# UltimateSoftware/surge

Measured on NVIDIA H100. Metric: events/sec replayed (segmented per-aggregate event fold), higher is better.
Workload: dtype i32

## Files before the change

### include/sgr.h

```cpp
#ifndef SGR_H
#define SGR_H

#include <stddef.h>
#include <stdint.h>

#ifdef __cplusplus
extern "C" {
#endif

#define SGR_ABI_VERSION 1

#define SGR_OK                 0
#define SGR_ERR_INVALID       -1
#define SGR_ERR_NO_DEVICE     -2
#define SGR_ERR_CUDA          -3
#define SGR_ERR_NO_PROGRAM    -4
#define SGR_ERR_NOT_LOADED    -5
#define SGR_ERR_UNSUPPORTED   -6
#define SGR_ERR_OOM           -7
#define SGR_ERR_STATE         -8
#define SGR_ERR_DIST          -9
#define SGR_ERR_CAPACITY     -10
#define SGR_ERR_AGAIN        -11

// ... 46 lines not shown

typedef struct sgr_engine sgr_engine;

typedef struct sgr_config {
  int32_t  device;
  uint32_t flags;
  uint64_t reserved[6];
} sgr_config;

typedef struct sgr_stats {
  uint64_t n_aggregates;
  uint64_t n_events;
  uint64_t event_bytes;
  uint64_t algorithmic_bytes;
  uint64_t n_errors;
  uint64_t n_long_segments;
  float    ms_h2d;
  float    ms_group;
  float    ms_fold;
  float    ms_d2h;
  uint32_t fold_launches;
  uint32_t head_plane;
  uint32_t plane_bytes;
  uint32_t reserved[5];
} sgr_stats;

int32_t sgr_abi_version(void);

int32_t sgr_create(const sgr_config* cfg, sgr_engine** out);
int32_t sgr_destroy(sgr_engine* e);
const char* sgr_last_error(const sgr_engine* e);

int32_t sgr_register_program(sgr_engine* e, const sgr_fold_program* prog);

int32_t sgr_load_events(sgr_engine* e, const void* events, uint64_t nbytes,
                        const uint64_t* seg_offsets, uint64_t n_agg);
int32_t sgr_load_events_device(sgr_engine* e, const void* d_events, uint64_t nbytes,
                               const uint64_t* d_seg_offsets, uint64_t n_agg);

int32_t sgr_load_events_indexed(sgr_engine* e, const void* events, uint64_t nbytes, const uint64_t* seg_offsets, uint64_t n_agg,
                                const uint64_t* rec_offsets, uint64_t n_records);
int32_t sgr_load_events_indexed_device(sgr_engine* e, const void* d_events, uint64_t nbytes, const uint64_t* d_seg_offsets,
                                       uint64_t n_agg, const uint64_t* d_rec_offsets, uint64_t n_records);

int32_t sgr_load_unsorted(sgr_engine* e, const void* records, uint64_t n_records, uint64_t n_agg);
int32_t sgr_load_unsorted_device(sgr_engine* e, const void* d_records, uint64_t n_records, uint64_t n_agg);

// ... 180 lines not shown
```

### surge_b200/csrc/engine.cu

```cuda
#include <cuda_runtime.h>
#include <stdarg.h>
#include <stdio.h>
#include <string.h>

#include <atomic>
#include <memory>
#include <mutex>
#include <string>
#include <vector>

#include "../../include/sgr.h"
#include "bulk_fold.cuh"
#include "changes.cuh"
#include "devbuf.h"
#include "dist.cuh"
#include "engine_internal.h"
#include "fold_kernels.cuh"
#include "fold_rows.cuh"
#include "group_kernels.cuh"
#include "id_index.cuh"
#include "id_order.cuh"
#include "incremental.cuh"
#include "keytable.h"
#include "put_batch.cuh"
// ... 16 lines not shown
constexpr size_t kCtlDup = 0, kCtlNoSlot = 1, kCtlGatherBad = 2, kCtlCut = 4, kCtlRange = 8, kPayloadOff = 96;

struct FlaggedRows {
  enum Kind { kWholeTable, kNothing, kHostList, kDeviceList };
  Kind kind = kWholeTable;
  uint64_t n = 0;
  uint32_t upper = 0;
  int next = 0;
  void forget() { kind = kWholeTable; }
  void nothing() { kind = kNothing; }
  void host_list(uint64_t count) { kind = kHostList; n = count; }
  void device_list(uint32_t bound) { kind = kDeviceList; upper = bound; next ^= 1; }
};

struct PendingFold {
  enum Kernel { kSequential, kRows, kRuns, kVarRuns };
  Kernel kernel = kSequential;
  bool stamped = false;
  bool prior = false;
  uint64_t n_seg = 0, event_bytes = 0;
  const uint8_t* events = nullptr; const uint64_t* offsets = nullptr; const uint32_t* ids = nullptr;
  const void* counters = nullptr;
  uint32_t plane = 0;
};
}

struct sgr_engine {
  int device = 0;
  int num_sms = 0;
  Stream stream;
  Event ev0, ev1;

  bool has_program = false;
  sgr_fold_program program{};
  DevProgram dprog{};

  DevBuf own_events, own_offsets, own_rec_offsets;
  const uint64_t* d_rec_offsets = nullptr;
  uint64_t n_rec = 0;
  const uint8_t* d_events = nullptr;
  const uint64_t* d_offsets = nullptr;
  uint64_t event_bytes = 0;
  uint64_t n_agg = 0;
  bool loaded = false;
  uint32_t max_record_bytes = 64;

  DevBuf states;
  bool states_valid = false;
  uint64_t states_n = 0;
  DevBuf counters;
  GroupScratch group;
  DevBuf inc_records, inc_offsets, inc_ids, inc_prev_ids;
  DevBuf inc_scratch, inc_touched[2], inc_err_ids, inc_counters;
  uint64_t inc_scratch_slots = 0;
  FlaggedRows flagged;

  bool row_ok = false;
  RowProgram row_prog{};
  int row_max_grid = 0;
  int run_max_grid = 0, run_max_grid_variant = -2, run_max_grid_plane = -2;
  int64_t opt_run_variant = -1;
  DevBuf part_flags, part_data, redo_ids;
  DevBuf run_counters;
  int run_counter_idx = 0;
  int64_t opt_run_chunk_bytes = 131072;
  uint32_t epoch = 0;
  size_t part_flags_cap_seen = 0;
  bool offsets_aligned64 = false;
  uint64_t log_begin = 0, log_end = 0, max_seg_bytes = 0;
  DevBuf head_plane;
  enum PlaneState { kPlaneNone, kPlaneValid, kPlaneNoMemory } plane_state = kPlaneNone;
  uint32_t plane_bytes = 0;
  int64_t opt_head_plane = 1;
  int64_t opt_head_variant = -1;
  int64_t opt_proj_variant = 0;
  Stream side_stream;
  Event ev_copied, ev_split;
  bool fold_pending = false;
  PendingFold pending;
  Event ev2, ev3;

  int64_t opt_kernel = 0;
  int64_t opt_variant = -1;
  int64_t opt_var_stages = 1;
  int64_t opt_var_stage_bytes = 12288;
  int64_t opt_replay_budget = 1ll << 24;
  int64_t opt_force_route = 0;
  int64_t opt_incremental = 0;
  int64_t opt_max_record_bytes = 528;

  bool bulk_ok = false;
  BulkLayout bulk_lay{};
  DevBuf bulk_scratch, bulk_err_ids, bulk_counters, hash_out;
  uint64_t bulk_scratch_slots = 0;
  int64_t opt_bulk = 1;
  int64_t opt_push_ordered = 0;
  int64_t opt_push_chunks = 16;

// ... 113 lines not shown
  return SGR_OK;
}

int32_t refresh_snapshot(sgr_engine* e, std::shared_ptr<Snapshot>* out) {
  std::lock_guard<std::recursive_mutex> g(e->op_mu);
  if (!e->snapshot_dirty.load(std::memory_order_acquire) && e->snapshot) { *out = e->snapshot; return SGR_OK; }
  const uint64_t gen = e->generation.load(std::memory_order_acquire);
  if (!e->states_valid) return fail(e, SGR_ERR_STATE, "state store is not readable: no fold has completed");
  int32_t rc = use_device(e); if (rc) return rc;
  rc = finish_fold(e); if (rc) return rc;
  auto s = std::make_shared<Snapshot>();
  s->n_agg = e->states_n; s->state_bytes = e->program.state_bytes;
  s->states.resize((size_t)s->n_agg * s->state_bytes);
  CUDA_TRY(e, cudaMemcpyAsync(s->states.data(), e->states.p, s->states.size(), cudaMemcpyDeviceToHost, e->stream));
  CUDA_TRY(e, cudaStreamSynchronize(e->stream));
  std::atomic_store(&e->snapshot, s);
  if (e->generation.load(std::memory_order_acquire) == gen) e->snapshot_dirty.store(false, std::memory_order_release);
  *out = s;
  return SGR_OK;
}

constexpr uint64_t kRedoCap = 1u << 20;

int32_t begin_lookback(sgr_engine* e, uint64_t n_warps_max, uint64_t words) {
  CUDA_TRY(e, e->part_flags.reserve(n_warps_max * 4 + 256));
  CUDA_TRY(e, e->part_data.reserve(n_warps_max * words * 4 + 256));
  CUDA_TRY(e, e->redo_ids.reserve(kRedoCap * 4));
  if (e->epoch == 0 || e->part_flags_cap_seen != e->part_flags.cap) {
    CUDA_TRY(e, cudaMemsetAsync(e->part_flags.p, 0, e->part_flags.cap, e->stream));
    e->part_flags_cap_seen = e->part_flags.cap;
  }
  ++e->epoch;
  if (e->epoch == 0) { CUDA_TRY(e, cudaMemsetAsync(e->part_flags.p, 0, e->part_flags.cap, e->stream)); e->epoch = 1; }
  return SGR_OK;
}

int32_t launch_replay(sgr_engine* e, const uint8_t* d_events, const uint64_t* d_offsets, const uint32_t* d_ids, const uint8_t* states_in,
                      unsigned long long* counters) {
  FoldArgs a{};
  a.events = d_events; a.seg_offsets = d_offsets; a.seg_ids = d_ids; a.n_seg = kRedoCap; a.seg_list = (const uint32_t*)e->redo_ids.p;
  a.n_seg_dev = counters + 3; a.states_in = states_in; a.states_out = (uint8_t*)e->states.p; a.counters = counters;
  FoldLaunchInfo info{};
  cudaError_t le = launch_fold_stream(a, e->dprog, -1, 8, e->max_record_bytes, e->stream, &info);
  if (le != cudaSuccess) return fail(e, SGR_ERR_CUDA, "replay launch: %s", cudaGetErrorString(le));
  return SGR_OK;
}

bool plane_wanted(const sgr_engine* e) {
  return e->row_ok && e->row_prog.head_only && e->opt_head_plane && e->opt_kernel == 0 && e->opt_run_variant < 0 &&
         e->program.record_kind == SGR_REC_FIXED64 && e->offsets_aligned64 && e->log_end > e->log_begin;
}

uint32_t plane_record_bytes(const sgr_engine* e) { return slot_plane_fits(e->row_prog) && e->opt_head_variant < 0 ? 16u : 32u; }

cudaError_t build_plane(sgr_engine* e, const uint8_t* log, uint32_t rec, uint64_t r0, uint64_t r1, cudaStream_t st) {
  uint8_t* p = (uint8_t*)e->head_plane.p;
  return rec == 16 ? launch_build_slots(log, p, r0, r1, e->row_prog, e->num_sms, st) : launch_build_heads(log, p, r0, r1, e->num_sms, st);
}

int32_t ensure_plane(sgr_engine* e, uint32_t* plane, bool* built) {
  const uint32_t rec = plane_record_bytes(e);
  *plane = 0; *built = false;
  if (e->plane_bytes != rec) e->plane_state = sgr_engine::kPlaneNone;
  if (e->plane_state == sgr_engine::kPlaneValid) *plane = rec;
  if (e->plane_state != sgr_engine::kPlaneNone) return SGR_OK;
  e->plane_bytes = rec;
  const uint64_t n_rec = (e->log_end - e->log_begin) / 64;
  if (e->fold_pending && e->head_plane.cap < n_rec * rec) CUDA_TRY(e, cudaStreamSynchronize(e->stream));
  if (e->head_plane.reserve(n_rec * rec) != cudaSuccess) {
    (void)cudaGetLastError();
    e->plane_state = sgr_engine::kPlaneNoMemory;
    return SGR_OK;
  }
  cudaError_t le = build_plane(e, e->d_events + e->log_begin, rec, 0, n_rec, e->stream);
  if (le != cudaSuccess) return fail(e, SGR_ERR_CUDA, "plane build: %s", cudaGetErrorString(le));
  e->plane_state = sgr_engine::kPlaneValid;
  *plane = rec; *built = true;
  return SGR_OK;
}

int32_t enqueue_fold(sgr_engine* e, const uint8_t* d_events, const uint64_t* d_offsets, const uint32_t* d_ids,
                     uint64_t n_seg, bool use_prior, uint64_t event_bytes, bool aligned64, uint64_t log_begin, uint64_t log_end) {
  const uint8_t* states_in = use_prior ? (const uint8_t*)e->states.p : nullptr;
  const bool wide_balanced = e->row_prog.user_words == 14 && e->opt_kernel == 0 && d_offsets == e->d_offsets && e->max_seg_bytes <= (256u << 10);
  bool use_rows = e->row_ok && !wide_balanced && e->program.record_kind == SGR_REC_FIXED64 && aligned64 && e->opt_kernel != 1 && n_seg < (1ull << 32) && n_seg > 0;
  if ((e->opt_kernel == 2 || e->opt_kernel == 3) && !use_rows && n_seg > 0)
    return fail(e, SGR_ERR_UNSUPPORTED, "record-parallel kernel cannot take this program/log");
  if (use_rows && e->opt_kernel == 3 && (e->row_prog.user_words != 2 || e->row_prog.cls != 0 || e->row_prog.n_slots > 6 || e->row_prog.f64_mask))
    return fail(e, SGR_ERR_UNSUPPORTED, "the record-per-lane kernel takes 16-byte class-0 programs only");
  const bool runs = use_rows && e->opt_kernel != 3;
  uint32_t plane = 0;
  bool plane_built = false;
  if (runs && plane_wanted(e) && d_events == e->d_events && d_offsets == e->d_offsets && !d_ids) {
    int32_t rc = ensure_plane(e, &plane, &plane_built); if (rc) return rc;
  }
  unsigned long long* counters = (unsigned long long*)e->counters.p;
  if (runs) {
    if (!e->run_counters.p) {
      CUDA_TRY(e, e->run_counters.reserve(256));
      CUDA_TRY(e, cudaMemsetAsync(e->run_counters.p, 0, 256, e->stream));
    }
    counters = (unsigned long long*)e->run_counters.p + 16 * e->run_counter_idx;
  } else {
    CUDA_TRY(e, cudaMemsetAsync(e->counters.p, 0, 64, e->stream));
  }
  const bool overlap = runs && !plane_built && e->fold_pending && e->pending.kernel == PendingFold::kRuns && e->pending.events == d_events &&
                       e->pending.offsets == d_offsets && e->pending.ids == d_ids && e->pending.plane == plane;
  if (!overlap) CUDA_TRY(e, cudaEventRecord(e->ev0, e->stream));
  uint32_t launches = 0;
  PendingFold::Kernel kernel = PendingFold::kSequential;
  const bool use_var = e->row_ok && e->row_prog.user_words == 2 && e->row_prog.cls == 0 && e->program.record_kind == SGR_REC_VAR16 && e->d_rec_offsets && d_offsets == e->d_offsets && !use_prior &&
                       !d_ids && e->opt_kernel != 1 && n_seg > 0 && n_seg < (1ull << 32) && e->n_rec > 0;
  if (use_var) {
    int threads = 0; size_t smem = 0; uint32_t stage = 0;
    const int max_grid = vruns_config(e->num_sms, e->max_record_bytes, (uint32_t)e->opt_var_stage_bytes, (int)e->opt_var_stages, &threads, &smem, &stage);
    if (max_grid > 0) {
      int32_t rc = begin_lookback(e, (uint64_t)max_grid * (threads / 32), 8); if (rc) return rc;
      CUDA_TRY(e, cudaMemsetAsync(e->states.p, 0, (size_t)n_seg * e->program.state_bytes, e->stream));
      VarArgs v{};
      v.events = d_events; v.rec_offsets = e->d_rec_offsets; v.n_rec = e->n_rec; v.seg_offsets = d_offsets; v.n_seg = n_seg;
      v.states_out = (uint8_t*)e->states.p; v.counters = counters; v.redo_ids = (uint32_t*)e->redo_ids.p; v.redo_cap = kRedoCap;
      v.part_flags = (uint32_t*)e->part_flags.p; v.part_data = (uint32_t*)e->part_data.p; v.epoch = e->epoch; v.stage_bytes = stage;
      v.max_record_bytes = e->max_record_bytes;
      const uint64_t steps = (e->n_rec + 31) / 32;
      uint64_t want = (steps + (threads / 32) - 1) / (threads / 32);
      const int grid = (int)(want < (uint64_t)max_grid ? want : (uint64_t)max_grid);
      cudaError_t le = launch_fold_vruns(v, e->row_prog, (int)e->opt_var_stages, grid, threads, smem, e->stream);
      if (le != cudaSuccess) return fail(e, SGR_ERR_CUDA, "fold_vruns launch: %s", cudaGetErrorString(le));
      rc = launch_replay(e, d_events, d_offsets, d_ids, states_in, counters); if (rc) return rc;
      launches = 2;
      kernel = PendingFold::kVarRuns;
    }
  }
  if (n_seg && kernel != PendingFold::kVarRuns) {
    if (use_rows) {
      const bool v1 = e->opt_kernel == 3;
      const int rv = plane == 16 ? (int)e->opt_proj_variant : plane == 32 ? (e->opt_head_variant < 0 ? 0 : (int)e->opt_head_variant)
                                                                          : (int)e->opt_run_variant;
      const int pl = (int)plane;
      if (v1 && !e->row_max_grid) e->row_max_grid = row_kernel_max_grid(e->num_sms, e->row_prog);
      if (!v1 && (e->run_max_grid_variant != rv || e->run_max_grid_plane != pl)) {
        e->run_max_grid = run_kernel_max_grid(e->num_sms, rv, pl, e->row_prog); e->run_max_grid_variant = rv; e->run_max_grid_plane = pl;
      }
      const int max_grid = v1 ? e->row_max_grid : e->run_max_grid;
      const int wpc = v1 ? kRowThreads / 32 : run_warps_per_cta();
      const uint64_t step_bytes = v1 ? 2048 : (uint64_t)run_variant_step_bytes(rv, pl, e->row_prog);
      const uint64_t steps = (log_end - log_begin + step_bytes - 1) / step_bytes;
      const uint64_t chunk_steps = v1 ? 1 : run_variant_chunk_steps(rv, pl, e->row_prog, (uint64_t)e->opt_run_chunk_bytes, steps, (uint64_t)max_grid * wpc);
      const uint64_t n_chunks = (steps + chunk_steps - 1) / chunk_steps;
      const uint64_t n_parts = v1 ? (uint64_t)max_grid * wpc : n_chunks;
      int32_t rc = begin_lookback(e, n_parts, e->row_prog.user_words + 2); if (rc) return rc;
      RowArgs r{};
      r.events = d_events; r.heads = plane ? (const uint8_t*)e->head_plane.p : nullptr; r.seg_offsets = d_offsets; r.seg_ids = d_ids; r.n_seg = n_seg;
      r.log_begin = log_begin; r.log_end = log_end;
      r.states_in = states_in; r.states_out = (uint8_t*)e->states.p;
      r.counters = counters;
      r.counters_next = runs ? (unsigned long long*)e->run_counters.p + 16 * (e->run_counter_idx ^ 1) : nullptr;
      r.redo_ids = (uint32_t*)e->redo_ids.p; r.redo_cap = kRedoCap;
      r.part_flags = (uint32_t*)e->part_flags.p; r.part_data = (uint32_t*)e->part_data.p; r.epoch = e->epoch;
      r.chunk_steps = chunk_steps;
      uint64_t want = (n_chunks + wpc - 1) / wpc;
      if (want == 0) want = 1;
      const int grid = (int)(want < (uint64_t)max_grid ? want : (uint64_t)max_grid);
      cudaError_t le = v1 ? launch_fold_rows(r, e->row_prog, grid, e->stream) : launch_fold_runs(r, e->row_prog, rv, pl, grid, overlap, e->stream);
      if (le != cudaSuccess) return fail(e, SGR_ERR_CUDA, "fold launch: %s", cudaGetErrorString(le));
      if (runs) {
        e->run_counter_idx ^= 1;
        launches = 1;
      } else {
        rc = launch_replay(e, d_events, d_offsets, d_ids, states_in, counters); if (rc) return rc;
        launches = 2;
      }
      kernel = runs ? PendingFold::kRuns : PendingFold::kRows;
    } else {
      FoldArgs a{};
      a.events = d_events; a.seg_offsets = d_offsets; a.seg_ids = d_ids; a.n_seg = n_seg;
      a.states_in = states_in; a.states_out = (uint8_t*)e->states.p;
      a.counters = counters;
      FoldLaunchInfo info{};
      cudaError_t le = launch_fold_stream(a, e->dprog, (int)e->opt_variant, e->num_sms, e->max_record_bytes, e->stream, &info);
      if (le == cudaErrorNotSupported || le == cudaErrorInvalidConfiguration)
        return fail(e, SGR_ERR_UNSUPPORTED, "fold_variant %lld cannot take this program at max_record_bytes %u (%s)",
                    (long long)e->opt_variant, e->max_record_bytes, cudaGetErrorString(le));
      if (le != cudaSuccess) return fail(e, SGR_ERR_CUDA, "fold launch: %s", cudaGetErrorString(le));
      launches = 1;
    }
  }
  if (!overlap) CUDA_TRY(e, cudaEventRecord(e->ev1, e->stream));
  e->fold_pending = true;
  e->pending = PendingFold{kernel, overlap, use_prior, n_seg, event_bytes, d_events, d_offsets, d_ids, counters, plane};
  e->stats.fold_launches = launches;
  e->stats.head_plane = plane ? 1u : 0u;
  e->stats.plane_bytes = plane;
  return SGR_OK;
}

int32_t finish_fold(sgr_engine* e) {
  if (!e->fold_pending) return SGR_OK;
  e->fold_pending = false;
  PendingFold& p = e->pending;
  unsigned long long h[16] = {};
  CUDA_TRY(e, cudaMemcpyAsync(h, p.counters, p.kernel == PendingFold::kRuns ? 128 : 64, cudaMemcpyDeviceToHost, e->stream));
  CUDA_TRY(e, cudaStreamSynchronize(e->stream));
  if (p.stamped) e->stats.ms_fold = (h[8] && h[9] > ~h[8]) ? (float)((double)(h[9] - ~h[8]) * 1e-6) : 0.f;
  else CUDA_TRY(e, cudaEventElapsedTime(&e->stats.ms_fold, e->ev0, e->ev1));
  if ((p.kernel == PendingFold::kVarRuns && h[7]) || (p.kernel != PendingFold::kSequential && h[3] > kRedoCap)) {
    if (p.prior) {
      e->states_valid = false; mark_dirty(e);
      return fail(e, SGR_ERR_UNSUPPORTED, "replay list overflow on an in-place incremental fold: state table invalidated, rebuild it");
    }
    FoldArgs a{};
    a.events = p.events; a.seg_offsets = p.offsets; a.seg_ids = p.ids; a.n_seg = p.n_seg;
    a.states_out = (uint8_t*)e->states.p; a.counters = (unsigned long long*)e->counters.p;
    CUDA_TRY(e, cudaMemsetAsync(e->counters.p, 0, 64, e->stream));
    CUDA_TRY(e, cudaEventRecord(e->ev2, e->stream));
    FoldLaunchInfo info{};
// ... 59 lines not shown
  *out = e.release();
  return SGR_OK;
}

int32_t sgr_destroy(sgr_engine* e) {
  if (!e) return SGR_OK;
  cudaSetDevice(e->device);
  cudaStreamSynchronize(e->stream);
  delete e;
  return SGR_OK;
}

int32_t sgr_register_program(sgr_engine* e, const sgr_fold_program* prog) {
  OpLock op_lock(e);
  if (!e || !prog) return fail(e, SGR_ERR_INVALID, "null argument");
  DevProgram d;
  int32_t rc = compile_program(e, prog, &d);
  if (rc) return rc;
  e->program = *prog; e->dprog = d; e->has_program = true;
  e->row_ok = build_row_program(d, &e->row_prog);
  e->bulk_ok = e->row_ok && prog->record_kind == SGR_REC_FIXED64 && bulk_layout_for(e->row_prog, &e->bulk_lay);
  e->bulk_scratch_slots = 0;
  e->row_max_grid = 0; e->run_max_grid_variant = -2;
  e->plane_state = sgr_engine::kPlaneNone;
  e->states_valid = false; e->states_n = 0;
  e->writer.n = 0;
  e->writer_framing = SGR_VALUE_JSON;
  mark_dirty(e);
  return SGR_OK;
}

static int32_t before_load(sgr_engine* e) {
  int32_t rc = use_device(e); if (rc) return rc;
  return finish_fold(e);
}

struct Upload { void* dst; const void* src; size_t bytes; };

static int32_t upload_timed(sgr_engine* e, cudaEvent_t t0, cudaEvent_t t1, std::initializer_list<Upload> uploads) {
  CUDA_TRY(e, cudaEventRecord(t0, e->stream));
  for (const Upload& u : uploads) CUDA_TRY(e, cudaMemcpyAsync(u.dst, u.src, u.bytes, cudaMemcpyHostToDevice, e->stream));
  CUDA_TRY(e, cudaEventRecord(t1, e->stream));
  CUDA_TRY(e, cudaStreamSynchronize(e->stream));
  CUDA_TRY(e, cudaEventElapsedTime(&e->stats.ms_h2d, t0, t1));
  return SGR_OK;
}

static int32_t after_load(sgr_engine* e, const uint8_t* d_events, const uint64_t* d_offsets, uint64_t nbytes, uint64_t n_agg) {
  e->d_events = d_events; e->d_offsets = d_offsets; e->event_bytes = nbytes; e->n_agg = n_agg; e->loaded = true;
  e->d_rec_offsets = nullptr; e->n_rec = 0;
  e->max_record_bytes = e->program.record_kind == SGR_REC_VAR16 ? (uint32_t)e->opt_max_record_bytes : 64u;
  e->offsets_aligned64 = false; e->log_begin = 0; e->log_end = nbytes;
  e->plane_state = sgr_engine::kPlaneNone;
  if (e->program.record_kind == SGR_REC_FIXED64) {
    cudaError_t ce = inspect_offsets(d_offsets, n_agg, (unsigned long long*)e->counters.p, e->stream, &e->offsets_aligned64,
                                     &e->log_begin, &e->log_end, &e->max_seg_bytes);
    if (ce != cudaSuccess) return fail(e, SGR_ERR_CUDA, "offset inspection: %s", cudaGetErrorString(ce));
  }
  return SGR_OK;
}

int32_t sgr_load_events(sgr_engine* e, const void* events, uint64_t nbytes, const uint64_t* seg_offsets, uint64_t n_agg) {
  OpLock op_lock(e);
  if (!e || (!events && nbytes) || !seg_offsets) return fail(e, SGR_ERR_INVALID, "null argument");
  if (!e->has_program) return fail(e, SGR_ERR_NO_PROGRAM, "register a fold program before loading events");
  if (seg_offsets[n_agg] > nbytes) return fail(e, SGR_ERR_INVALID, "seg_offsets[n_agg]=%llu exceeds nbytes=%llu",
                                               (unsigned long long)seg_offsets[n_agg], (unsigned long long)nbytes);
  for (uint64_t i = 0; i <= n_agg; ++i) {
    if (seg_offsets[i] % 16) return fail(e, SGR_ERR_INVALID, "seg_offsets[%llu] is not a multiple of 16", (unsigned long long)i);
    if (i && seg_offsets[i] < seg_offsets[i - 1]) return fail(e, SGR_ERR_INVALID, "seg_offsets not monotone at %llu", (unsigned long long)i);
  }
  int32_t rc = before_load(e); if (rc) return rc;
  CUDA_TRY(e, e->own_events.reserve(nbytes));
  CUDA_TRY(e, e->own_offsets.reserve((n_agg + 1) * 8));
  const uint64_t begin = seg_offsets[0], end = seg_offsets[n_agg];
  bool aligned64 = true;
// ... 1493 lines not shown
```

### surge_b200/csrc/fold_rows.cuh

```cuda
#pragma once
#include <cuda_runtime.h>
#include <stdint.h>
#include <string.h>

#include "../../include/sgr.h"
#include "sgr_device.cuh"

namespace sgr {

constexpr int kRowThreads = 256;
constexpr int kMaxSlots = 16;
constexpr int kMaxRowWords = 14;
constexpr int kTabStride = 16;

constexpr uint32_t kRuleValid = 1u;
constexpr uint32_t kRuleNone = 2u;
constexpr uint32_t kRuleIfExists = 4u;
constexpr uint32_t kRuleNew = 8u;
constexpr uint32_t kModeAdd = 1u, kModeSet = 2u;

__host__ __device__ __forceinline__ uint32_t spec_encode(uint32_t mode, uint32_t neg, uint32_t slot) { return mode | (neg << 2) | (slot << 3); }
__host__ __device__ __forceinline__ uint32_t spec_mode(uint32_t spec) { return spec & 3u; }
__host__ __device__ __forceinline__ uint32_t spec_slot(uint32_t spec) { return spec >> 3; }
__host__ __device__ __forceinline__ bool spec_neg(uint32_t spec) { return (spec & 4u) != 0u; }
// ... 12 lines not shown
  uint32_t f64_mask;
  uint32_t head_only;
  uint32_t slot_word[kMaxSlots];
  uint32_t tab[16 * kTabStride];
};

struct RowArgs {
  const uint8_t* events;
  const uint8_t* heads;
  const uint64_t* seg_offsets;
  const uint32_t* seg_ids;
  uint64_t n_seg;
  uint64_t log_begin, log_end;
  const uint8_t* states_in;
  uint8_t* states_out;
  unsigned long long* counters;
  unsigned long long* counters_next;
  uint32_t* redo_ids;
  uint64_t redo_cap;
  uint32_t* part_flags;
  uint32_t* part_data;
  uint32_t epoch;
  uint64_t chunk_steps;
};

bool build_row_program(const DevProgram& dp, RowProgram* out);
struct WordModes {
  uint32_t add, set;
  bool none;
};
WordModes word_modes(const RowProgram& prog);

template <int W>
__device__ __forceinline__ void finish_row(uint8_t* row, const uint32_t (&old)[W], uint32_t ex0, const uint32_t (&nw)[W], uint32_t exn) {
  uint32_t outw[W + 2], changed = exn != ex0;
#pragma unroll
  for (int w = 0; w < W; ++w) {
    outw[w] = exn ? nw[w] : 0u;
    if (exn && ex0) changed |= (outw[w] != old[w]);
  }
  outw[W] = exn | (changed ? SGR_ST_CHANGED : 0u);
  outw[W + 1] = 0u;
  uint4* dp = reinterpret_cast<uint4*>(row);
#pragma unroll
  for (int q = 0; q < (W + 2) / 4; ++q) dp[q] = make_uint4(outw[4 * q], outw[4 * q + 1], outw[4 * q + 2], outw[4 * q + 3]);
}
// ... 15 lines not shown
  uint64_t n_rec;
  const uint64_t* seg_offsets;
  uint64_t n_seg;
  uint8_t* states_out;
  unsigned long long* counters;
  uint32_t* redo_ids; uint64_t redo_cap;
  uint32_t* part_flags; uint32_t* part_data; uint32_t epoch;
  uint32_t stage_bytes;
  uint32_t max_record_bytes;
};
int vruns_config(int num_sms, uint32_t max_record_bytes, uint32_t stage_hint, int nstage, int* threads, size_t* smem, uint32_t* stage_bytes);
cudaError_t launch_fold_vruns(const VarArgs& args, const RowProgram& prog, int nstage, int grid, int threads, size_t smem, cudaStream_t stream);

int run_variant_count();
const char* run_variant_name(int v);
int head_variant_count();
int proj_variant_count();
bool slot_plane_fits(const RowProgram& prog);
int run_kernel_max_grid(int num_sms, int variant, int plane, const RowProgram& prog);
int run_variant_step_bytes(int variant, int plane, const RowProgram& prog);
int run_warps_per_cta();
uint64_t run_variant_chunk_steps(int variant, int plane, const RowProgram& prog, uint64_t chunk_bytes, uint64_t steps, uint64_t n_warps);
cudaError_t launch_fold_runs(const RowArgs& args, const RowProgram& prog, int variant, int plane, int grid, bool overlap, cudaStream_t stream);
cudaError_t launch_build_heads(const uint8_t* log, uint8_t* heads, uint64_t rec0, uint64_t rec1, int num_sms, cudaStream_t stream);
cudaError_t launch_build_slots(const uint8_t* log, uint8_t* slots, uint64_t rec0, uint64_t rec1, const RowProgram& prog, int num_sms,
                               cudaStream_t stream);

}
```

### surge_b200/csrc/fold_runs.cu

```cuda
#include <stdio.h>

#include "../../include/sgr.h"
#include "fold_rows.cuh"

namespace sgr {
namespace {

constexpr int kRunThreads = 128;
constexpr int kRunWarps = kRunThreads / 32;

template <int W>
struct Xf {
  uint32_t m;
  uint32_t ex;
  uint32_t v[W];
};

template <int W>
__device__ __forceinline__ Xf<W> identity() {
  Xf<W> r;
  r.m = 0; r.ex = 0;
#pragma unroll
  for (int w = 0; w < W; ++w) r.v[w] = 0;
  return r;
// ... 86 lines not shown
    const uint4* sp = reinterpret_cast<const uint4*>(a.states_in + slot * (uint64_t)(W + 2) * 4);
#pragma unroll
    for (int q = 0; q < (W + 2) / 4; ++q) {
      uint4 v4 = __ldg(sp + q);
      if (q == (W + 2) / 4 - 1) { v4.z &= SGR_ST_EXISTS; v4.w = 0u; }
      dp[q] = v4;
    }
  } else {
#pragma unroll
    for (int q = 0; q < (W + 2) / 4; ++q) dp[q] = make_uint4(0, 0, 0, 0);
  }
}

template <int R, int NSTAGE, int REC = 64>
__host__ __device__ constexpr int warp_smem_bytes() {
  return NSTAGE * 32 * REC * R
         + 2 * 32 * R * 4
         + 32 * 4;
}

template <int W>
__device__ __noinline__ void replay_segments(const RowArgs& a, const RowProgram& pg, const uint32_t* tab, int lane, unsigned long long n_redo);

template <int W, int CLS>
__device__ __forceinline__ Xf<W> look_back_chunks(const RowArgs& a, uint64_t c) {
  Xf<W> pre = identity<W>();
  while (c > 0) {
    --c;
    const uint32_t* pf = a.part_flags + c;
    while (ld_volatile_u32(pf) != a.epoch) { __nanosleep(64); }
    __threadfence();
    const uint32_t* pd = a.part_data + c * (W + 2);
    Xf<W> e;
    e.m = ld_volatile_u32(pd);
#pragma unroll
    for (int w = 0; w < W; ++w) e.v[w] = ld_volatile_u32(pd + 1 + w);
    const uint32_t tailw = ld_volatile_u32(pd + W + 1);
    e.ex = tailw & 3u;
    pre = compose<W, CLS>(e, pre);
    if (tailw & 4u) break;
  }
  return pre;
}

template <int W, int R, int NSTAGE, int NS, int MINB, bool DIRECT, int CLS, int REC = 64>
__global__ void __launch_bounds__(kRunThreads, MINB) fold_runs_kernel(const __grid_constant__ RowArgs a, const __grid_constant__ RowProgram pg) {
  static_assert(R % 2 == 0 && 8 % R == 0, "R in {2,4,8}");
  static_assert(REC == 64 || REC == 32 || REC == 16, "the log, the head plane or the slot plane");
  static_assert(R * REC >= 128, "a lane's run starts on a 128-byte line: R >= 128 / REC");
  static_assert(REC != 16 || (!DIRECT && NS == 4), "the slot plane holds four slot words, not record words");
  constexpr int STEP_BYTES = 2048 * R;
// ... 77 lines not shown
    nxt = n_warps + t < n_chunks ? n_warps + t : kNone;
    nxt_pending = false;
  };
  int ist = 0;
  auto issue_next = [&]() {
    if (iss == iss_end && iss_chunk != kNone) {
      resolve_next();
      if (nxt != kNone && nxt != iss_chunk) {
        iss_chunk = nxt; iss = nxt * cs; iss_end = iss + cs < total_steps ? iss + cs : total_steps;
      }
    }
    if (iss < iss_end) {
      issue_step(iss, ist);
      ++iss;
      if (++ist == NSTAGE) ist = 0;
    }
  };

#pragma unroll
  for (int s = 0; s < NSTAGE - 1; ++s) {
    issue_next();
    cp_async_commit();
  }
  uint64_t kc = (chunk != kNone && chunk != 0) ? first_boundary(base + chunk * cs * STEP_BYTES) : 0;

  constexpr int NSOFF = DIRECT ? 1 : NS;
  constexpr int SOFF_RPL = REC == 16 ? 1 : RPL;
  uint32_t soff[SOFF_RPL][NSOFF];
  if constexpr (REC != 16) {
#pragma unroll
    for (int s = 0; s < NSOFF; ++s) {
      const uint32_t c = pg.slot_word[s] >> 2, k = pg.slot_word[s] & 3u;
#pragma unroll
      for (int rl = 0; rl < RPL; ++rl) soff[rl][s] = ((((uint32_t)(CPR * rl) + c) ^ (uint32_t)(lane & 7)) << 4) + (k << 2);
    }
  }
  uint64_t win_b = ~0ull, win_bn = ~0ull;
  auto load_window = [&]() {
    const uint64_t k = kc + lane;
    win_b = k <= n_seg ? a.seg_offsets[k] : ~0ull;
    win_bn = k < n_seg ? a.seg_offsets[k + 1] : ~0ull;
  };
  if (chunk != kNone) load_window();

  grid_dep_wait();
  if (threadIdx.x == 0) atomicMax(a.counters + 8, ~t_entry);
  if (gw == 0 && lane < 16) a.counters_next[lane] = 0ull;
  auto look_back = [&](uint64_t c) -> Xf<W> { return look_back_chunks<W, CLS>(a, c); };
  bool dfr = false;
  uint64_t dfr_chunk = 0;
  uint32_t dfr_seg = 0;
  Xf<W> dfr_t = identity<W>();

  unsigned long long n_applied = 0;
  int stage = 0;
  uint64_t prev_chunk = kNone;
  while (chunk != kNone) {
    const uint64_t step0 = chunk * cs;
    const uint64_t step_end = step0 + cs < total_steps ? step0 + cs : total_steps;
    const uint64_t wb = base + step0 * STEP_BYTES;
    if (iss_chunk != chunk) { iss_chunk = chunk; iss = step0; iss_end = step_end; }
    if (lane == 0) tk = atomicAdd(a.counters + 10, 1ull);
    nxt_pending = true;
    if (prev_chunk != kNone && chunk != prev_chunk + 1) {
      kc = chunk != 0 ? first_boundary(wb) : 0;
      load_window();
    }

    bool span_has_head = false;
    bool inh_pending = false;
    uint32_t inh_seg = 0;
    Xf<W> inh_t = identity<W>();
    Xf<W> carry = identity<W>();

    for (uint64_t step = step0; step < step_end; ++step) {
      issue_next();
      cp_async_commit();
      const uint64_t sb = base + step * (uint64_t)STEP_BYTES;
      const uint64_t rem = a.log_end - sb;
      const uint32_t span = rem < (uint64_t)STEP_BYTES ? (uint32_t)rem : (uint32_t)STEP_BYTES;
      const int nvalid = (int)(span >> 6);

#pragma unroll
      for (int i = 0; i < R; ++i) { hs_end[i * 32 + lane] = 0xffffffffu; hs_start[i * 32 + lane] = 0u; }
      if (lane < R) hmask[lane] = 0u;
      __syncwarp();
      while (true) {
        const uint64_t k = kc + lane;
        const uint64_t b = win_b, bn = win_bn;
        const uint64_t d = b - sb;
// ... 90 lines not shown
        const uint32_t window = (lane_heads >> sh) & ((1u << dd) - 1u);
        if (lane >= dd && window == 0) sc = compose<W, CLS>(o, sc);
      }
      Xf<W> cin = shfl_xf(sc, lane - 1);
      if (lane == 0) cin = carry;
      carry = shfl_xf(sc, 31);

      if (have_first && first_seg != 0xffffffffu) {
        const Xf<W> tot = compose<W, CLS>(cin, first);
        const bool is_span_first = !span_has_head && (lane_heads & ((1u << lane) - 1u)) == 0;
        if (is_span_first && chunk != 0) { inh_t = tot; inh_seg = first_seg; inh_pending = true; }
        else finish_segment<W>(a, f64_mask, first_seg, tot);
      }
      if (lane_heads) {
        if (!span_has_head) {
          const int src = __ffs(lane_heads) - 1;
          inh_t = shfl_xf(inh_t, src);
          inh_seg = __shfl_sync(0xffffffffu, inh_seg, src);
          inh_pending = __shfl_sync(0xffffffffu, (int)inh_pending, src) != 0;
        }
        span_has_head = true;
      }
      __syncwarp();
      if (++stage == NSTAGE) stage = 0;
    }

    bool end_needs_lookback = false;
    if (step_end == total_steps) {
      for (uint64_t k = kc + lane; k < n_seg; k += 32) finish_empty<W>(a, (uint32_t)k);
      if (kc >= 1) {
        if (span_has_head || chunk == 0) { if (lane == 0) finish_segment<W>(a, f64_mask, (uint32_t)(kc - 1), carry); }
        else end_needs_lookback = true;
      }
    }

    {
      uint32_t* part_data = a.part_data + chunk * (W + 2);
      if (lane == 0) {
        part_data[0] = carry.m;
#pragma unroll
        for (int w = 0; w < W; ++w) part_data[1 + w] = carry.v[w];
        part_data[W + 1] = carry.ex | (span_has_head ? 4u : 0u);
        __threadfence();
        st_volatile_u32(a.part_flags + chunk, a.epoch);
      }
      if (lane == 0) {
        if (dfr) { finish_segment<W>(a, f64_mask, dfr_seg, compose<W, CLS>(look_back(dfr_chunk), dfr_t)); dfr = false; }
        if (inh_pending) { dfr = true; dfr_chunk = chunk; dfr_seg = inh_seg; dfr_t = inh_t; }
        if (end_needs_lookback) finish_segment<W>(a, f64_mask, (uint32_t)(kc - 1), compose<W, CLS>(look_back(chunk), carry));
      }
      __syncwarp();
    }
    {
      const uint64_t we = base + step_end * (uint64_t)STEP_BYTES < a.log_end ? base + step_end * (uint64_t)STEP_BYTES : a.log_end;
      n_applied += (we - wb) >> 6;
    }
    prev_chunk = chunk;
    resolve_next();
    chunk = nxt;
  }
  cp_async_wait<0>();
// ... 209 lines not shown
      const uint32_t sw = (sel >> (4 * s)) & 7u;
      uint32_t v = 0;
#pragma unroll
      for (int k = 0; k < 8; ++k) v = sw == (uint32_t)k ? w[k] : v;
      o[s] = (uint32_t)s < n_slots ? v : 0u;
    }
    reinterpret_cast<uint4*>(slots)[r] = make_uint4(o[0], o[1], o[2], o[3]);
  }
}

cudaError_t launch_build_slots(const uint8_t* log, uint8_t* slots, uint64_t rec0, uint64_t rec1, const RowProgram& prog, int num_sms,
                               cudaStream_t stream) {
  if (rec1 <= rec0) return cudaSuccess;
  if (!slot_plane_fits(prog)) return cudaErrorInvalidValue;
  uint32_t sel = 0;
  bool upper = false;
  for (uint32_t s = 0; s < prog.n_slots; ++s) { sel |= prog.slot_word[s] << (4 * s); upper |= prog.slot_word[s] >= 4; }
  const uint64_t want = (rec1 - rec0 + 255) / 256;
  const uint64_t cap = (uint64_t)num_sms * 16;
  build_slots_kernel<<<(unsigned)(want < cap ? want : cap), 256, 0, stream>>>(log, slots, rec0, rec1, sel, prog.n_slots, upper);
  return cudaGetLastError();
}

namespace {
template <bool TICKET>
__global__ void __launch_bounds__(kRunThreads, 3) read_probe_kernel(const uint8_t* buf, uint64_t bytes, uint64_t chunk_steps, unsigned long long* ctl) {
  constexpr int R = 4, NSTAGE = 2, STEP_BYTES = 2048 * R;
  extern __shared__ __align__(128) uint8_t smem_raw[];
  const int lane = threadIdx.x & 31, warp = threadIdx.x >> 5;
  const uint32_t stage0 = smem_u32(smem_raw + (size_t)warp * warp_smem_bytes<R, NSTAGE>());
  const uint64_t gw = (uint64_t)blockIdx.x * kRunWarps + warp, n_warps = (uint64_t)gridDim.x * kRunWarps;
  const uint64_t total_steps = (bytes + STEP_BYTES - 1) / STEP_BYTES;
  auto issue = [&](uint64_t s, int stage) {
    const uint64_t sbyte = s * (uint64_t)STEP_BYTES;
    const uint32_t dst = stage0 + (uint32_t)stage * STEP_BYTES + (uint32_t)lane * 16u;
#pragma unroll
    for (int q = 0; q < 4 * R; ++q)
      if (sbyte + (uint64_t)q * 512 + (uint64_t)lane * 16 < bytes) cp_async16(dst + q * 512, buf + sbyte + q * 512 + lane * 16);
  };
  uint32_t acc = 0;
  auto run = [&](uint64_t s0, uint64_t s1) {
    if (s0 < s1) issue(s0, 0);
    cp_async_commit();
    int stage = 0;
    for (uint64_t s = s0; s < s1; ++s) {
      if (s + 1 < s1) issue(s + 1, stage ^ 1);
// ... 42 lines not shown
```

### surge_b200/native.py

```python
from __future__ import annotations

import ctypes as C
import os
from typing import Optional

from . import build as _build

SGR_OK = 0
ERR_NAMES = {
    -1: "SGR_ERR_INVALID", -2: "SGR_ERR_NO_DEVICE", -3: "SGR_ERR_CUDA", -4: "SGR_ERR_NO_PROGRAM",
    -5: "SGR_ERR_NOT_LOADED", -6: "SGR_ERR_UNSUPPORTED", -7: "SGR_ERR_OOM", -8: "SGR_ERR_STATE",
    -9: "SGR_ERR_DIST", -10: "SGR_ERR_CAPACITY", -11: "SGR_ERR_AGAIN",
}
SGR_ERR_INVALID, SGR_ERR_NO_DEVICE, SGR_ERR_CUDA, SGR_ERR_NO_PROGRAM, SGR_ERR_NOT_LOADED = -1, -2, -3, -4, -5
SGR_ERR_UNSUPPORTED, SGR_ERR_OOM, SGR_ERR_STATE, SGR_ERR_DIST, SGR_ERR_CAPACITY = -6, -7, -8, -9, -10
SGR_ERR_AGAIN = -11

REC_FIXED64, REC_VAR16 = 0, 1
ST_EXISTS, ST_CHANGED, ST_ERROR = 1, 2, 4
MAX_STATE_BYTES, MAX_TYPES, MAX_OPS = 128, 16, 8
IF_EXISTS, MATERIALISE, CREATE, TOMBSTONE, THROW = 0, 1, 2, 3, 4
OP_SET, OP_ADD_I32, OP_SUB_I32, OP_ADD_I64, OP_SUB_I64 = 0, 1, 2, 3, 4


# ... 19 lines not shown


class sgr_fold_program(C.Structure):
    _fields_ = [("state_bytes", C.c_uint32), ("record_kind", C.c_uint32), ("n_types", C.c_uint32),
                ("n_f64_fields", C.c_uint32), ("f64_field_off", C.c_uint16 * 8), ("rules", sgr_rule * MAX_TYPES)]


class sgr_config(C.Structure):
    _fields_ = [("device", C.c_int32), ("flags", C.c_uint32), ("reserved", C.c_uint64 * 6)]


class sgr_dist_stats(C.Structure):
    _fields_ = [("n_sent", C.c_uint64), ("n_sent_remote", C.c_uint64), ("n_recv", C.c_uint64), ("n_local_aggregates", C.c_uint64),
                ("ms_count", C.c_float), ("ms_counts_exchange", C.c_float), ("ms_scatter", C.c_float), ("ms_exchange", C.c_float),
                ("ms_group", C.c_float), ("ms_fold", C.c_float), ("ms_pipeline", C.c_float), ("exchange_record_bytes", C.c_uint32),
                ("reserved", C.c_uint32 * 4)]


class sgr_stats(C.Structure):
    _fields_ = [("n_aggregates", C.c_uint64), ("n_events", C.c_uint64), ("event_bytes", C.c_uint64),
                ("algorithmic_bytes", C.c_uint64), ("n_errors", C.c_uint64), ("n_long_segments", C.c_uint64),
                ("ms_h2d", C.c_float), ("ms_group", C.c_float), ("ms_fold", C.c_float), ("ms_d2h", C.c_float),
                ("fold_launches", C.c_uint32), ("head_plane", C.c_uint32), ("plane_bytes", C.c_uint32),
                ("reserved", C.c_uint32 * 5)]


class sgr_changes_cursor(C.Structure):
    _fields_ = [("next", C.c_uint64), ("token", C.c_uint64), ("n_keys", C.c_uint64), ("reserved", C.c_uint64)]


class sgr_ingest_stats(C.Structure):
    _fields_ = [(n, C.c_uint64) for n in ("n_bytes", "n_trailing_bytes", "n_batches", "n_records", "n_markers", "n_null_values",
                                          "n_control_batches", "n_aborted_batches", "n_aborted_records", "n_duplicates", "n_new_keys",
                                          "n_compressed_bytes", "n_decompressed_bytes")] + [("reserved", C.c_uint64 * 3)]


class sgr_json_field(C.Structure):
    _fields_ = [("name", C.c_char_p), ("kind", C.c_uint8), ("reserved", C.c_uint8), ("dst_off", C.c_uint16), ("len", C.c_uint32)]


class sgr_json_event(C.Structure):
    _fields_ = [("type_name", C.c_char_p), ("event_type", C.c_uint32), ("n_fields", C.c_uint32), ("fields", sgr_json_field * 8)]


JSON_I32, JSON_I64, JSON_F64, JSON_UUID, JSON_PSTR = 0, 1, 2, 3, 4
JSON_ID = 5
VALUE_PACKED, VALUE_PROTOBUF_EVENT, VALUE_JSON, VALUE_PROTOBUF_JSON = 0, 1, 2, 3
# ... 135 lines not shown
```

Before: 143.7 billion.

## Precompute chunk-to-segment table and pack look-back rows into single vector stores

Adds a precomputed per-chunk first-segment table, built once by a binary-search kernel and cached on the engine. For the 16-byte head plane path, the run kernel now reads each chunk's starting segment from this table instead of doing a binary search per chunk, and it prefetches the next chunk's segment window while still working on the current chunk. The look-back partition record (carry mask, exists bits, head flag, two state words and epoch) is packed into one 16-byte volatile vector store and load. This removes the separate flag/data reads and the thread fence. The cost is extra memory for the table, an extra kernel launch whenever the table is rebuilt, and a layout restricted to W==2.

After: 152.1 billion, median of 6. 1.06x the previous value.

```diff
diff --git a/include/sgr.h b/include/sgr.h
--- a/include/sgr.h
+++ b/include/sgr.h
@@ -92,7 +92,8 @@
   uint32_t fold_launches;
   uint32_t head_plane;
   uint32_t plane_bytes;
-  uint32_t reserved[5];
+  uint32_t chunk_table;
+  uint32_t reserved[4];
 } sgr_stats;
 
 int32_t sgr_abi_version(void);
diff --git a/surge_b200/csrc/engine.cu b/surge_b200/csrc/engine.cu
--- a/surge_b200/csrc/engine.cu
+++ b/surge_b200/csrc/engine.cu
@@ -62,6 +62,7 @@
   const uint8_t* events = nullptr; const uint64_t* offsets = nullptr; const uint32_t* ids = nullptr;
   const void* counters = nullptr;
   uint32_t plane = 0;
+  const void* chunk_table = nullptr;
 };
 }
 
@@ -106,6 +107,7 @@
   int64_t opt_run_chunk_bytes = 131072;
   uint32_t epoch = 0;
   size_t part_flags_cap_seen = 0;
+  bool part_flags_rows = false;
   bool offsets_aligned64 = false;
   uint64_t log_begin = 0, log_end = 0, max_seg_bytes = 0;
   DevBuf head_plane;
@@ -114,6 +116,8 @@
   int64_t opt_head_plane = 1;
   int64_t opt_head_variant = -1;
   int64_t opt_proj_variant = 0;
+  DevBuf chunk_table;
+  uint64_t chunk_table_steps = 0, chunk_table_step_bytes = 0;
   Stream side_stream;
   Event ev_copied, ev_split;
   bool fold_pending = false;
@@ -273,16 +277,18 @@
 
 constexpr uint64_t kRedoCap = 1u << 20;
 
-int32_t begin_lookback(sgr_engine* e, uint64_t n_warps_max, uint64_t words) {
-  CUDA_TRY(e, e->part_flags.reserve(n_warps_max * 4 + 256));
+int32_t begin_lookback(sgr_engine* e, uint64_t n_warps_max, uint64_t words, bool rows = false) {
+  CUDA_TRY(e, e->part_flags.reserve(n_warps_max * (rows ? 16 : 4) + 256));
   CUDA_TRY(e, e->part_data.reserve(n_warps_max * words * 4 + 256));
   CUDA_TRY(e, e->redo_ids.reserve(kRedoCap * 4));
-  if (e->epoch == 0 || e->part_flags_cap_seen != e->part_flags.cap) {
+  if (e->epoch == 0 || e->part_flags_cap_seen != e->part_flags.cap || (e->part_flags_rows && !rows)) {
     CUDA_TRY(e, cudaMemsetAsync(e->part_flags.p, 0, e->part_flags.cap, e->stream));
     e->part_flags_cap_seen = e->part_flags.cap;
-  }
+    e->part_flags_rows = false;
+  }
+  e->part_flags_rows |= rows;
   ++e->epoch;
-  if (e->epoch == 0) { CUDA_TRY(e, cudaMemsetAsync(e->part_flags.p, 0, e->part_flags.cap, e->stream)); e->epoch = 1; }
+  if (e->epoch == 0) { CUDA_TRY(e, cudaMemsetAsync(e->part_flags.p, 0, e->part_flags.cap, e->stream)); e->epoch = 1; e->part_flags_rows = rows; }
   return SGR_OK;
 }
 
@@ -327,6 +333,25 @@
   if (le != cudaSuccess) return fail(e, SGR_ERR_CUDA, "plane build: %s", cudaGetErrorString(le));
   e->plane_state = sgr_engine::kPlaneValid;
   *plane = rec; *built = true;
+  return SGR_OK;
+}
+
+int32_t ensure_chunk_table(sgr_engine* e, const uint64_t* d_offsets, uint64_t n_seg, uint64_t log_begin, uint64_t step_bytes,
+                           uint64_t chunk_steps, uint64_t n_chunks, const uint64_t** table, bool* built) {
+  *table = nullptr; *built = false;
+  if (e->chunk_table_steps != chunk_steps || e->chunk_table_step_bytes != step_bytes) {
+    e->chunk_table_steps = 0;
+    if (e->fold_pending && e->chunk_table.cap < n_chunks * 8) CUDA_TRY(e, cudaStreamSynchronize(e->stream));
+    if (e->chunk_table.reserve(n_chunks * 8) != cudaSuccess) {
+      (void)cudaGetLastError();
+      return SGR_OK;
+    }
+    cudaError_t le = launch_build_chunk_table(d_offsets, n_seg, log_begin, step_bytes, chunk_steps, n_chunks, (uint64_t*)e->chunk_table.p, e->stream);
+    if (le != cudaSuccess) return fail(e, SGR_ERR_CUDA, "chunk table build: %s", cudaGetErrorString(le));
+    e->chunk_table_steps = chunk_steps; e->chunk_table_step_bytes = step_bytes;
+    *built = true;
+  }
+  *table = (const uint64_t*)e->chunk_table.p;
   return SGR_OK;
 }
 
@@ -346,6 +371,25 @@
     int32_t rc = ensure_plane(e, &plane, &plane_built); if (rc) return rc;
   }
   unsigned long long* counters = (unsigned long long*)e->counters.p;
+  const uint64_t* chunk_table = nullptr;
+  bool table_built = false;
+  const int rv = plane == 16 ? (int)e->opt_proj_variant : plane == 32 ? (e->opt_head_variant < 0 ? 0 : (int)e->opt_head_variant)
+                                                                      : (int)e->opt_run_variant;
+  uint64_t chunk_steps = 0;
+  if (runs && n_seg) {
+    const int pl = (int)plane;
+    if (e->run_max_grid_variant != rv || e->run_max_grid_plane != pl) {
+      e->run_max_grid = run_kernel_max_grid(e->num_sms, rv, pl, e->row_prog); e->run_max_grid_variant = rv; e->run_max_grid_plane = pl;
+    }
+    const uint64_t step_bytes = (uint64_t)run_variant_step_bytes(rv, pl, e->row_prog);
+    const uint64_t steps = (log_end - log_begin + step_bytes - 1) / step_bytes;
+    chunk_steps = run_variant_chunk_steps(rv, pl, e->row_prog, (uint64_t)e->opt_run_chunk_bytes, steps, (uint64_t)e->run_max_grid * run_warps_per_cta());
+    if (plane == 16) {
+      int32_t rc = ensure_chunk_table(e, d_offsets, n_seg, log_begin, step_bytes, chunk_steps, (steps + chunk_steps - 1) / chunk_steps,
+                                      &chunk_table, &table_built);
+      if (rc) return rc;
+    }
+  }
   if (runs) {
     if (!e->run_counters.p) {
       CUDA_TRY(e, e->run_counters.reserve(256));
@@ -355,8 +399,9 @@
   } else {
     CUDA_TRY(e, cudaMemsetAsync(e->counters.p, 0, 64, e->stream));
   }
-  const bool overlap = runs && !plane_built && e->fold_pending && e->pending.kernel == PendingFold::kRuns && e->pending.events == d_events &&
-                       e->pending.offsets == d_offsets && e->pending.ids == d_ids && e->pending.plane == plane;
+  const bool overlap = runs && !plane_built && !table_built && e->fold_pending && e->pending.kernel == PendingFold::kRuns &&
+                       e->pending.events == d_events && e->pending.offsets == d_offsets && e->pending.ids == d_ids && e->pending.plane == plane &&
+                       e->pending.chunk_table == chunk_table;
   if (!overlap) CUDA_TRY(e, cudaEventRecord(e->ev0, e->stream));
   uint32_t launches = 0;
   PendingFold::Kernel kernel = PendingFold::kSequential;
@@ -386,21 +431,16 @@
   if (n_seg && kernel != PendingFold::kVarRuns) {
     if (use_rows) {
       const bool v1 = e->opt_kernel == 3;
-      const int rv = plane == 16 ? (int)e->opt_proj_variant : plane == 32 ? (e->opt_head_variant < 0 ? 0 : (int)e->opt_head_variant)
-                                                                          : (int)e->opt_run_variant;
       const int pl = (int)plane;
       if (v1 && !e->row_max_grid) e->row_max_grid = row_kernel_max_grid(e->num_sms, e->row_prog);
-      if (!v1 && (e->run_max_grid_variant != rv || e->run_max_grid_plane != pl)) {
-        e->run_max_grid = run_kernel_max_grid(e->num_sms, rv, pl, e->row_prog); e->run_max_grid_variant = rv; e->run_max_grid_plane = pl;
-      }
       const int max_grid = v1 ? e->row_max_grid : e->run_max_grid;
       const int wpc = v1 ? kRowThreads / 32 : run_warps_per_cta();
       const uint64_t step_bytes = v1 ? 2048 : (uint64_t)run_variant_step_bytes(rv, pl, e->row_prog);
       const uint64_t steps = (log_end - log_begin + step_bytes - 1) / step_bytes;
-      const uint64_t chunk_steps = v1 ? 1 : run_variant_chunk_steps(rv, pl, e->row_prog, (uint64_t)e->opt_run_chunk_bytes, steps, (uint64_t)max_grid * wpc);
+      if (v1) chunk_steps = 1;
       const uint64_t n_chunks = (steps + chunk_steps - 1) / chunk_steps;
       const uint64_t n_parts = v1 ? (uint64_t)max_grid * wpc : n_chunks;
-      int32_t rc = begin_lookback(e, n_parts, e->row_prog.user_words + 2); if (rc) return rc;
+      int32_t rc = begin_lookback(e, n_parts, e->row_prog.user_words + 2, !v1 && plane == 16); if (rc) return rc;
       RowArgs r{};
       r.events = d_events; r.heads = plane ? (const uint8_t*)e->head_plane.p : nullptr; r.seg_offsets = d_offsets; r.seg_ids = d_ids; r.n_seg = n_seg;
       r.log_begin = log_begin; r.log_end = log_end;
@@ -409,7 +449,7 @@
       r.counters_next = runs ? (unsigned long long*)e->run_counters.p + 16 * (e->run_counter_idx ^ 1) : nullptr;
       r.redo_ids = (uint32_t*)e->redo_ids.p; r.redo_cap = kRedoCap;
       r.part_flags = (uint32_t*)e->part_flags.p; r.part_data = (uint32_t*)e->part_data.p; r.epoch = e->epoch;
-      r.chunk_steps = chunk_steps;
+      r.chunk_steps = chunk_steps; r.chunk_kc = chunk_table;
       uint64_t want = (n_chunks + wpc - 1) / wpc;
       if (want == 0) want = 1;
       const int grid = (int)(want < (uint64_t)max_grid ? want : (uint64_t)max_grid);
@@ -439,10 +479,11 @@
   }
   if (!overlap) CUDA_TRY(e, cudaEventRecord(e->ev1, e->stream));
   e->fold_pending = true;
-  e->pending = PendingFold{kernel, overlap, use_prior, n_seg, event_bytes, d_events, d_offsets, d_ids, counters, plane};
+  e->pending = PendingFold{kernel, overlap, use_prior, n_seg, event_bytes, d_events, d_offsets, d_ids, counters, plane, chunk_table};
   e->stats.fold_launches = launches;
   e->stats.head_plane = plane ? 1u : 0u;
   e->stats.plane_bytes = plane;
+  e->stats.chunk_table = chunk_table ? 1u : 0u;
   return SGR_OK;
 }
 
@@ -548,7 +589,7 @@
   e->bulk_ok = e->row_ok && prog->record_kind == SGR_REC_FIXED64 && bulk_layout_for(e->row_prog, &e->bulk_lay);
   e->bulk_scratch_slots = 0;
   e->row_max_grid = 0; e->run_max_grid_variant = -2;
-  e->plane_state = sgr_engine::kPlaneNone;
+  e->plane_state = sgr_engine::kPlaneNone; e->chunk_table_steps = 0;
   e->states_valid = false; e->states_n = 0;
   e->writer.n = 0;
   e->writer_framing = SGR_VALUE_JSON;
@@ -577,7 +618,7 @@
   e->d_rec_offsets = nullptr; e->n_rec = 0;
   e->max_record_bytes = e->program.record_kind == SGR_REC_VAR16 ? (uint32_t)e->opt_max_record_bytes : 64u;
   e->offsets_aligned64 = false; e->log_begin = 0; e->log_end = nbytes;
-  e->plane_state = sgr_engine::kPlaneNone;
+  e->plane_state = sgr_engine::kPlaneNone; e->chunk_table_steps = 0;
   if (e->program.record_kind == SGR_REC_FIXED64) {
     cudaError_t ce = inspect_offsets(d_offsets, n_agg, (unsigned long long*)e->counters.p, e->stream, &e->offsets_aligned64,
                                      &e->log_begin, &e->log_end, &e->max_seg_bytes);
diff --git a/surge_b200/csrc/fold_rows.cuh b/surge_b200/csrc/fold_rows.cuh
--- a/surge_b200/csrc/fold_rows.cuh
+++ b/surge_b200/csrc/fold_rows.cuh
@@ -58,6 +58,7 @@
   uint32_t* part_data;
   uint32_t epoch;
   uint64_t chunk_steps;
+  const uint64_t* chunk_kc;
 };
 
 bool build_row_program(const DevProgram& dp, RowProgram* out);
@@ -119,6 +120,8 @@
 int run_warps_per_cta();
 uint64_t run_variant_chunk_steps(int variant, int plane, const RowProgram& prog, uint64_t chunk_bytes, uint64_t steps, uint64_t n_warps);
 cudaError_t launch_fold_runs(const RowArgs& args, const RowProgram& prog, int variant, int plane, int grid, bool overlap, cudaStream_t stream);
+cudaError_t launch_build_chunk_table(const uint64_t* off, uint64_t n_seg, uint64_t log_begin, uint64_t step_bytes, uint64_t chunk_steps,
+                                     uint64_t n_chunks, uint64_t* table, cudaStream_t stream);
 cudaError_t launch_build_heads(const uint8_t* log, uint8_t* heads, uint64_t rec0, uint64_t rec1, int num_sms, cudaStream_t stream);
 cudaError_t launch_build_slots(const uint8_t* log, uint8_t* slots, uint64_t rec0, uint64_t rec1, const RowProgram& prog, int num_sms,
                                cudaStream_t stream);
diff --git a/surge_b200/csrc/fold_runs.cu b/surge_b200/csrc/fold_runs.cu
--- a/surge_b200/csrc/fold_runs.cu
+++ b/surge_b200/csrc/fold_runs.cu
@@ -132,11 +132,31 @@
 template <int W>
 __device__ __noinline__ void replay_segments(const RowArgs& a, const RowProgram& pg, const uint32_t* tab, int lane, unsigned long long n_redo);
 
-template <int W, int CLS>
+__device__ __forceinline__ uint4 ld_volatile_v4(const uint32_t* p) {
+  uint4 v;
+  asm volatile("ld.volatile.global.v4.u32 {%0,%1,%2,%3}, [%4];" : "=r"(v.x), "=r"(v.y), "=r"(v.z), "=r"(v.w) : "l"(p));
+  return v;
+}
+__device__ __forceinline__ void st_volatile_v4(uint32_t* p, uint32_t x, uint32_t y, uint32_t z, uint32_t w) {
+  asm volatile("st.volatile.global.v4.u32 [%0], {%1,%2,%3,%4};" ::"l"(p), "r"(x), "r"(y), "r"(z), "r"(w) : "memory");
+}
+constexpr uint32_t kRowEx = 4, kRowHead = 64u, kRowFields = 0x70u;
+
+template <int W, int CLS, bool PACKED = false>
 __device__ __forceinline__ Xf<W> look_back_chunks(const RowArgs& a, uint64_t c) {
   Xf<W> pre = identity<W>();
   while (c > 0) {
     --c;
+    if constexpr (PACKED) {
+      static_assert(W == 2, "a packed row holds two state words");
+      uint4 r = ld_volatile_v4(a.part_flags + 4 * c);
+      while (r.w != a.epoch) { __nanosleep(64); r = ld_volatile_v4(a.part_flags + 4 * c); }
+      Xf<W> e;
+      e.m = r.x & ~kRowFields; e.ex = (r.x >> kRowEx) & 3u; e.v[0] = r.y; e.v[1] = r.z;
+      pre = compose<W, CLS>(e, pre);
+      if (r.x & kRowHead) break;
+      continue;
+    }
     const uint32_t* pf = a.part_flags + c;
     while (ld_volatile_u32(pf) != a.epoch) { __nanosleep(64); }
     __threadfence();
@@ -260,7 +280,11 @@
     issue_next();
     cp_async_commit();
   }
-  uint64_t kc = (chunk != kNone && chunk != 0) ? first_boundary(base + chunk * cs * STEP_BYTES) : 0;
+  uint64_t kc = 0;
+  if (chunk != kNone && chunk != 0) {
+    if constexpr (REC == 16) kc = a.chunk_kc ? a.chunk_kc[chunk] : first_boundary(base + chunk * cs * STEP_BYTES);
+    else kc = first_boundary(base + chunk * cs * STEP_BYTES);
+  }
 
   constexpr int NSOFF = DIRECT ? 1 : NS;
   constexpr int SOFF_RPL = REC == 16 ? 1 : RPL;
@@ -280,11 +304,14 @@
     win_bn = k < n_seg ? a.seg_offsets[k + 1] : ~0ull;
   };
   if (chunk != kNone) load_window();
+  uint32_t pf_kc = ~0u;
+  uint64_t pf_b = ~0ull, pf_bn = ~0ull;
+  bool pf_win = false;
 
   grid_dep_wait();
   if (threadIdx.x == 0) atomicMax(a.counters + 8, ~t_entry);
   if (gw == 0 && lane < 16) a.counters_next[lane] = 0ull;
-  auto look_back = [&](uint64_t c) -> Xf<W> { return look_back_chunks<W, CLS>(a, c); };
+  auto look_back = [&](uint64_t c) -> Xf<W> { return look_back_chunks<W, CLS, REC == 16>(a, c); };
   bool dfr = false;
   uint64_t dfr_chunk = 0;
   uint32_t dfr_seg = 0;
@@ -301,9 +328,17 @@
     if (lane == 0) tk = atomicAdd(a.counters + 10, 1ull);
     nxt_pending = true;
     if (prev_chunk != kNone && chunk != prev_chunk + 1) {
-      kc = chunk != 0 ? first_boundary(wb) : 0;
-      load_window();
-    }
+      bool have_win = false;
+      if constexpr (REC == 16) {
+        if (!a.chunk_kc) kc = first_boundary(wb);
+        else if (pf_win) { kc = pf_kc; win_b = pf_b; win_bn = pf_bn; have_win = true; }
+        else kc = pf_kc != ~0u ? pf_kc : a.chunk_kc[chunk];
+      } else {
+        kc = chunk != 0 ? first_boundary(wb) : 0;
+      }
+      if (!have_win) load_window();
+    }
+    pf_kc = ~0u; pf_win = false;
 
     bool span_has_head = false;
     bool inh_pending = false;
@@ -440,6 +475,17 @@
         span_has_head = true;
       }
       __syncwarp();
+      if constexpr (REC == 16) {
+        if (a.chunk_kc && pf_kc == ~0u) {
+          resolve_next();
+          if (nxt != kNone && nxt != chunk + 1) pf_kc = (uint32_t)a.chunk_kc[nxt];
+        } else if (a.chunk_kc && !pf_win) {
+          const uint64_t k = (uint64_t)pf_kc + lane;
+          pf_b = k <= n_seg ? a.seg_offsets[k] : ~0ull;
+          pf_bn = k < n_seg ? a.seg_offsets[k + 1] : ~0ull;
+          pf_win = true;
+        }
+      }
       if (++stage == NSTAGE) stage = 0;
     }
 
@@ -453,8 +499,12 @@
     }
 
     {
-      uint32_t* part_data = a.part_data + chunk * (W + 2);
-      if (lane == 0) {
+      if constexpr (REC == 16) {
+        if (lane == 0)
+          st_volatile_v4(a.part_flags + 4 * chunk, carry.m | (carry.ex << kRowEx) | (span_has_head ? kRowHead : 0u), carry.v[0], carry.v[1],
+                         a.epoch);
+      } else if (lane == 0) {
+        uint32_t* part_data = a.part_data + chunk * (W + 2);
         part_data[0] = carry.m;
 #pragma unroll
         for (int w = 0; w < W; ++w) part_data[1 + w] = carry.v[w];
@@ -710,6 +760,26 @@
   return cudaGetLastError();
 }
 
+__global__ void __launch_bounds__(256) build_chunk_table_kernel(const uint64_t* off, uint64_t n_seg, uint64_t log_begin, uint64_t chunk_bytes,
+                                                               uint64_t n_chunks, uint64_t* table) {
+  const uint64_t c = (uint64_t)blockIdx.x * blockDim.x + threadIdx.x;
+  if (c >= n_chunks) return;
+  const uint64_t wb = log_begin + c * chunk_bytes;
+  uint64_t lo = 0, hi = n_seg + 1;
+  while (lo < hi) {
+    const uint64_t mid = lo + (hi - lo) / 2;
+    if (off[mid] >= wb) hi = mid; else lo = mid + 1;
+  }
+  table[c] = lo;
+}
+
+cudaError_t launch_build_chunk_table(const uint64_t* off, uint64_t n_seg, uint64_t log_begin, uint64_t step_bytes, uint64_t chunk_steps,
+                                     uint64_t n_chunks, uint64_t* table, cudaStream_t stream) {
+  if (!n_chunks) return cudaSuccess;
+  build_chunk_table_kernel<<<(unsigned)((n_chunks + 255) / 256), 256, 0, stream>>>(off, n_seg, log_begin, step_bytes * chunk_steps, n_chunks, table);
+  return cudaGetLastError();
+}
+
 namespace {
 template <bool TICKET>
 __global__ void __launch_bounds__(kRunThreads, 3) read_probe_kernel(const uint8_t* buf, uint64_t bytes, uint64_t chunk_steps, unsigned long long* ctl) {
diff --git a/surge_b200/native.py b/surge_b200/native.py
--- a/surge_b200/native.py
+++ b/surge_b200/native.py
@@ -65,7 +65,7 @@
                 ("algorithmic_bytes", C.c_uint64), ("n_errors", C.c_uint64), ("n_long_segments", C.c_uint64),
                 ("ms_h2d", C.c_float), ("ms_group", C.c_float), ("ms_fold", C.c_float), ("ms_d2h", C.c_float),
                 ("fold_launches", C.c_uint32), ("head_plane", C.c_uint32), ("plane_bytes", C.c_uint32),
-                ("reserved", C.c_uint32 * 5)]
+                ("chunk_table", C.c_uint32), ("reserved", C.c_uint32 * 4)]
 
 
 class sgr_changes_cursor(C.Structure):
```
